# JiangongChen/ORB_SLAM3-1

Measured on AMD Instinct MI355X. Metric: tracking frames/s (ORB extract+match), higher is better.
Workload: dtype u8; 1 GPU; ORBextractor 640x480, 8 levels, 1000 features (configs[1]) + SearchByBoW 1000x1000 per frame (configs[2]); batch_per_gpu=256

## Files before the change

orb_slam3-1_amd/csrc/orbx_extractor.hip:

```cpp
#include <hip/hip_runtime.h>

#include <algorithm>
#include <cmath>
#include <cstdarg>
#include <cstdio>
#include <cstdlib>
#include <cstring>
#include <string>
#include <vector>

#include "hip_check.h"
#include "orbx_kernels.hip"

namespace orbx {

thread_local std::string g_last_error;

int fail(int code, const char* fmt, ...)
{
    char buf[512];
    va_list ap;
    va_start(ap, fmt);
    vsnprintf(buf, sizeof(buf), fmt, ap);
    va_end(ap);
// ... 37 lines not shown
        return ORBX_OK;
    }
    int upload(const std::vector<T>& v)
    {
        int r = ensure(v.size() ? v.size() : 1);
        if (r) return r;
        if (!v.empty()) ORBX_HIP(hipMemcpy(p, v.data(), v.size() * sizeof(T), hipMemcpyHostToDevice));
        return ORBX_OK;
    }
    void release() { if (p) (void)hipFree(p); p = nullptr; n = 0; }
};

}

using namespace orbx;

struct orbx_extractor {
    int device = 0;
    int nfeatures = 0, nlevels = 0, ini_th = 0, min_th = 0;
    float scale_factor_f = 0;
    double scale_factor_d = 0;
    std::vector<float> scale, inv_scale, sigma2, inv_sigma2;
    std::vector<int> nfeat;
    int taps[7];
    int max_kp = 0;

    int geo_w = 0, geo_h = 0;
    std::vector<LevelDesc> levels;
    std::vector<CellDesc> cells;
    std::vector<TileDesc> tiles;
    size_t pyr_frame_bytes = 0;
    int cand_frame_entries = 0, sel_frame_entries = 0;
    std::vector<StripDesc> strips;
    FastLds fast_layout;
    int fast_corner_cap = 0;
    size_t fast_lds = 0, oct_lds = 0;
    int oct_pool = 0, oct_lds_keys = 0, oct_small_keys = 0;
    bool oct_nodes_hbm = false;
    size_t oct_node_stride = 0;
    size_t oct_small_lds = 0;
    int oct_dyn_keys = 0;
    size_t oct_dyn_lds = 0;
    bool oct_keys_forced = false;

    DevBuf<LevelDesc> d_levels;
    DevBuf<CellDesc> d_cells;
    DevBuf<TileDesc> d_tiles;
    DevBuf<StripDesc> d_strips;
    std::vector<DevBuf<int> > d_qsx0;
    std::vector<DevBuf<uint4> > d_qsel, d_qalpha;
    std::vector<DevBuf<ResizeRow> > d_rows;
    std::vector<DevBuf<int> > d_xofs, d_yofs;
    std::vector<DevBuf<short> > d_ialpha, d_ibeta;
    std::vector<uint8_t> resize_generic;

    int batch_cap = 0, last_batch = 0;
    DevBuf<uint8_t> d_pyr, d_blur;
    DevBuf<uint32_t> d_cand, d_scratch, d_sel;
    DevBuf<uint8_t> d_oct_nodes;
    DevBuf<int> d_cell_count, d_sel_count, d_kp_dst;
    DevBuf<OrbxKeyPoint> d_lvl_kps;
    DevBuf<OrbxKeyPoint> d_kps;
    DevBuf<uint8_t> d_desc;
    DevBuf<int> d_n, d_mono, d_status;
    DevBuf<int> d_sad;
    DevBuf<uint8_t> d_stereo_io;
    int out_cap = 0;
    hipStream_t stream = nullptr;
    static constexpr int kProfEvents = 8;
    bool profile = false;
    hipEvent_t prof_ev[kProfEvents] = {};
    int prof_marks = 0;
    hipStream_t prof_stream = nullptr;
    hipStream_t side_stream = nullptr;
    hipEvent_t ev_fork = nullptr, ev_join = nullptr;
    hipStream_t oct_stream = nullptr;
    hipEvent_t ev_oct_join = nullptr, ev_fast0 = nullptr, ev_resize = nullptr;
    hipEvent_t ev_tail = nullptr;
    int dbg_tail_delay_us = 0;
    int last_octree_variant = 0;
    int oct_split = 0, oct_pool_hi = 0;
// ... 20 lines not shown
{
    const int nl = e->nlevels;
    e->scale.assign(nl, 1.0f); e->sigma2.assign(nl, 1.0f); e->inv_scale.resize(nl); e->inv_sigma2.resize(nl);
    for (int i = 1; i < nl; i++) {
        e->scale[i] = (float)(e->scale[i - 1] * e->scale_factor_d);
        e->sigma2[i] = e->scale[i] * e->scale[i];
    }
    for (int i = 0; i < nl; i++) {
        e->inv_scale[i] = 1.0f / e->scale[i];
        e->inv_sigma2[i] = 1.0f / e->sigma2[i];
    }
    e->nfeat.resize(nl);
    const float factor = (float)(1.0f / e->scale_factor_d);
    float per_scale = e->nfeatures * (1 - factor) / (1 - (float)std::pow((double)factor, (double)nl));
    int sum = 0;
    for (int l = 0; l < nl - 1; l++) {
        e->nfeat[l] = (int)std::nearbyintf(per_scale);
        sum += e->nfeat[l];
        per_scale *= factor;
    }
    e->nfeat[nl - 1] = std::max(e->nfeatures - sum, 0);
    e->max_kp = 0;
    for (int l = 0; l < nl; l++) e->max_kp += std::max(e->nfeat[l] + 3, 32);
    gauss_taps_q8(7, 2.0, e->taps);
}

int orbx_extractor::setup_geometry(int w, int h)
{
    if (w == geo_w && h == geo_h) return ORBX_OK;
    levels.assign(nlevels, LevelDesc());
    cells.clear();
    tiles.clear();
    strips.clear();
    size_t off = 0;
    int cand_off = 0, sel_off = 0, max_tw = 0, max_th = 0, max_nfeat = 0;
    std::vector<int> node_need(nlevels, 0);
    d_qsx0.resize(nlevels); d_yofs.resize(nlevels); d_qsel.resize(nlevels); d_qalpha.resize(nlevels); d_ibeta.resize(nlevels); d_rows.resize(nlevels);
    d_xofs.resize(nlevels); d_ialpha.resize(nlevels); resize_generic.assign(nlevels, 0);
    for (int l = 0; l < nlevels; l++) {
        LevelDesc& L = levels[l];
        L.w = (int)std::nearbyintf((float)w * inv_scale[l]);
        L.h = (int)std::nearbyintf((float)h * inv_scale[l]);
        if (L.w < 1 || L.h < 1) return fail(ORBX_ERR_ARG, "pyramid level %d of a %dx%d image is empty", l, w, h);
        if (L.w > 4096 + 32 || L.h > 4096 + 32) return fail(ORBX_ERR_ARG, "image %dx%d too large (keys are 12-bit)", w, h);
        L.stride = round_up(L.w, 64);
        L.off = (int64_t)off;
        off += (size_t)L.stride * L.h;
        off = (off + 255) & ~(size_t)255;
        L.nfeat = nfeat[l];
        L.scale = scale[l];
        L.patch_size = (int)(kPatch * scale[l]);
        {
            const int bw = (L.w - kEdge + 3) - (kEdge - 3), bh = (L.h - kEdge + 3) - (kEdge - 3);
            const int n_ini = bh > 0 ? (int)std::roundf((float)bw / (float)bh) : 0;
            L.sel_off = sel_off; L.sel_cap = std::max({nfeat[l] + 3, 32, 4 * std::max(n_ini, 0)});
            node_need[l] = std::max(nfeat[l], 4 * std::max(n_ini, 0));
        }
        sel_off += (L.sel_cap + 1) & ~1;
        max_nfeat = std::max(max_nfeat, node_need[l]);
        L.cell_begin = (int)cells.size();
        L.cand_off = cand_off;
        const int minBX = kEdge - 3, minBY = minBX, maxBX = L.w - kEdge + 3, maxBY = L.h - kEdge + 3;
        const float width = (float)(maxBX - minBX), height = (float)(maxBY - minBY);
        const int nCols = (int)(width / 35.f), nRows = (int)(height / 35.f);
        if (nCols > 0 && nRows > 0) {
            const int wCell = (int)std::ceil(width / nCols), hCell = (int)std::ceil(height / nRows);
// ... 99 lines not shown
                rows[dy].sy = (uint32_t)sy0 | ((uint32_t)sy1 << 16);
                rows[dy].b0 = (uint32_t)ib[2 * y] << 12; rows[dy].b1 = (uint32_t)ib[2 * y + 1] << 12; rows[dy].pad = 0;
            }
            int r;
            if (resize_generic[l] && ((r = d_xofs[l].upload(xofs)) || (r = d_ialpha[l].upload(ia)) || (r = d_yofs[l].upload(yofs)) || (r = d_ibeta[l].upload(ib)))) return r;
            if ((r = d_qsx0[l].upload(qsx0)) || (r = d_qsel[l].upload(qsel)) || (r = d_qalpha[l].upload(qal)) || (r = d_rows[l].upload(rows))) return r;
        }
    }
    pyr_frame_bytes = off;
    if (off >= ((size_t)1 << 31)) return fail(ORBX_ERR_ARG, "the pyramid of a %dx%d image exceeds 2 GiB per frame", w, h);
    cand_frame_entries = std::max(cand_off, 1);
    sel_frame_entries = sel_off;
    {
        if (cells.size() > 32767) return fail(ORBX_ERR_ARG, "%zu FAST cells exceed the strip table's 16-bit cell index", cells.size());
        int max_nch = 1, max_ngx = 1, max_sth = 7, max_ent = 1, max_ncell = 1, max_int = 1;
        for (const StripDesc& sd : strips) {
            const int g0 = (sd.x0 + 3) >> 2, g1 = (sd.x1 - 4) >> 2, ngx = g1 - g0 + 1, sth = sd.y1 - sd.y0, ih = sth - 6;
            if (ngx > 64 || ih > 127) return fail(ORBX_ERR_ARG, "FAST strip of %dx%d px exceeds the 64-quad x 127-row work item index", sd.x1 - sd.x0, sth);
            const int xa = (4 * (g0 - 1)) & ~15, qoff = 4 * g0 - xa;
            max_nch = std::max(max_nch, (qoff + 4 * ngx + 4 + 15) >> 4);
            for (int j = 0; j < sd.ncell; j++) { const CellDesc& c = cells[sd.cell0 + j]; max_int = std::max(max_int, (c.x1 - c.x0 - 6) * ih); }
            max_ngx = std::max(max_ngx, ngx); max_sth = std::max(max_sth, sth);
            max_ent = std::max(max_ent, ((ih + 3) / 4) * (ngx + sd.ncell - 1));
            max_ncell = std::max(max_ncell, (int)sd.ncell);
        }
        if (max_int > 8191) return fail(ORBX_ERR_ARG, "FAST cell interior of %d px exceeds the 8191-px bitmask", max_int);
        FastLds& Z = fast_layout;
        auto al16 = [](size_t v) { return (v + 15) & ~(size_t)15; };
        size_t o = 0;
        Z.tile_pitch = 16 * max_nch;
        o = al16((size_t)max_sth * Z.tile_pitch);
        Z.map_off = (int)o; Z.map_pitch = 4 * max_ngx + 8;
        o = al16(o + (size_t)(max_sth - 6 + 2) * Z.map_pitch);
        Z.colcell_off = (int)o; o = al16(o + Z.map_pitch);
        Z.ent_cap = (max_ent + 7) & ~7;
        Z.ent_off = (int)o; o = al16(o + 2 * 4 * (size_t)Z.ent_cap);
        Z.px_off = (int)o; o = al16(o + 2 * 4 * (size_t)kPxCap);
        Z.corner_cap = fast_corner_cap > 0 ? fast_corner_cap : kCornerCap;
        Z.corner_off = (int)o; o = al16(o + 2 * 4 * (size_t)Z.corner_cap);
        Z.wpc = (max_int + 31) / 32;
        Z.pre_off = (int)o; o = al16(o + 4 * (size_t)max_ncell * Z.wpc);
        Z.bits_off = (int)o; o = al16(o + 4 * (size_t)max_ncell * Z.wpc);
        Z.total = (int)o;
        fast_lds = o;
        if (fast_lds > 150 * 1024) return fail(ORBX_ERR_ARG, "FAST strip of %d quads x %d rows does not fit LDS", max_ngx, max_sth);
    }
    oct_pool = max_nfeat + 16;
    if (oct_pool > 32000) return fail(ORBX_ERR_ARG, "nfeatures per level %d too large for the device octree (16-bit node ids)", max_nfeat);
    const char* env = getenv("ORBX_OCT_LDS_KEYS");
    oct_lds_keys = env ? atoi(env) : 0;
    oct_keys_forced = env != nullptr;
    auto pool_bytes = [](int pool) { return (size_t)pool * (2 * sizeof(SortNode) + 8 + 16 + 2 * kOctLogFactor) + (size_t)((pool + 15) & ~15); };
    const size_t node_bytes = pool_bytes(oct_pool);
    oct_split = 0; oct_pool_hi = 0; oct_lds_hi = 0;
    {
        size_t best = (size_t)nlevels * node_bytes;
        for (int sp = 1; sp < nlevels; sp++) {
            int hi = 0;
            for (int l = sp; l < nlevels; l++) hi = std::max(hi, node_need[l]);
            const size_t cost = (size_t)sp * node_bytes + (size_t)(nlevels - sp) * pool_bytes(hi + 16);
            if (cost < best) { best = cost; oct_split = sp; oct_pool_hi = hi + 16; oct_lds_hi = pool_bytes(hi + 16) + 16; }
        }
    }
    oct_nodes_hbm = node_bytes > 150 * 1024;
    oct_node_stride = (node_bytes + 255) & ~(size_t)255;
    if (oct_nodes_hbm) oct_lds_keys = 0;
    if (!oct_nodes_hbm && node_bytes + 8 * (size_t)oct_lds_keys > 150 * 1024) oct_lds_keys = (int)((150 * 1024 - node_bytes) / 8);
    if (oct_lds_keys < 0) oct_lds_keys = 0;
    oct_lds = node_bytes + 8 * (size_t)oct_lds_keys + 16;
    int max_cand_cap = 0;
    for (const LevelDesc& lv : levels) max_cand_cap = std::max(max_cand_cap, lv.cand_cap);
    oct_small_keys = max_cand_cap;
    if (oct_nodes_hbm || node_bytes + 8 * (size_t)oct_small_keys > 150 * 1024) oct_small_keys = 0;
    oct_small_lds = node_bytes + 8 * (size_t)oct_small_keys + 16;
    if (oct_lds_keys > 0 && oct_lds_keys < max_cand_cap) oct_lds_keys = 0;
    oct_dyn_keys = 0; oct_dyn_lds = 0;
    if (!oct_nodes_hbm && oct_small_keys == 0 && node_bytes + 8 * 2048 <= 150 * 1024) {
        oct_dyn_keys = (int)std::min<size_t>((size_t)max_cand_cap, (150 * 1024 - node_bytes) / 8);
        if (const char* envd = getenv("ORBX_OCT_DYN_KEYS")) oct_dyn_keys = std::max(64, std::min(oct_dyn_keys, atoi(envd)));
        oct_dyn_lds = node_bytes + 8 * (size_t)oct_dyn_keys + 16;
    }
    if (!oct_nodes_hbm) {
        ORBX_HIP(hipFuncSetAttribute((const void*)k_octree<false>, hipFuncAttributeMaxDynamicSharedMemorySize, (int)node_bytes + 64));
        ORBX_HIP(hipFuncSetAttribute((const void*)k_octree<true>, hipFuncAttributeMaxDynamicSharedMemorySize, (int)std::max(oct_lds, oct_small_lds)));
        if (oct_dyn_keys > 0) ORBX_HIP(hipFuncSetAttribute((const void*)k_octree_dyn, hipFuncAttributeMaxDynamicSharedMemorySize, (int)oct_dyn_lds));
    } else {
        oct_lds = 64; oct_small_lds = 64;
    }
    ORBX_HIP(hipFuncSetAttribute((const void*)k_fast_strips, hipFuncAttributeMaxDynamicSharedMemorySize, (int)fast_lds));
    int r;
    if ((r = d_levels.upload(levels)) || (r = d_cells.upload(cells)) || (r = d_tiles.upload(tiles)) || (r = d_strips.upload(strips))) return r;
    geo_w = w; geo_h = h;
    batch_cap = 0;
    return ORBX_OK;
}

int orbx_extractor::ensure_batch(int batch)
{
    if (batch <= batch_cap) return ORBX_OK;
    int r;
    const size_t B = (size_t)batch;
    if ((r = d_pyr.ensure(B * pyr_frame_bytes + 64)) || (r = d_blur.ensure(B * pyr_frame_bytes + 64)) ||
        (r = d_cand.ensure(B * cand_frame_entries)) || (r = d_scratch.ensure(B * 2 * cand_frame_entries)) ||
        (r = d_sel.ensure(B * sel_frame_entries)) || (r = d_cell_count.ensure(B * std::max<size_t>(cells.size(), 1))) ||
        (r = d_sel_count.ensure(B * nlevels)) || (r = d_kp_dst.ensure(B * sel_frame_entries)) ||
        (r = d_lvl_kps.ensure(B * sel_frame_entries)) || (r = d_n.ensure(B)) || (r = d_mono.ensure(B)) || (r = d_status.ensure(B)))
        return r;
    if (oct_nodes_hbm && (r = d_oct_nodes.ensure(B * nlevels * oct_node_stride))) return r;
    ORBX_HIP(hipMemset(d_pyr.p, 0, B * pyr_frame_bytes + 64));
    ORBX_HIP(hipMemset(d_blur.p, 0, B * pyr_frame_bytes + 64));
    batch_cap = batch;
    return ORBX_OK;
}

namespace orbx {
__global__ void k_debug_spin(long long ticks)
{
    const long long t0 = wall_clock64();
    while (wall_clock64() - t0 < ticks) __builtin_amdgcn_s_sleep(32);
}
__global__ __launch_bounds__(256) void k_copy_level0(const uint8_t* __restrict__ src, int row_stride, size_t src_frame_stride,
                                                     uint8_t* __restrict__ pyr, size_t frame_stride, LevelDesc L)
{
    const int x4 = (blockIdx.x * blockDim.x + threadIdx.x) * 4;
    const int y = blockIdx.y;
    if (x4 >= L.w) return;
    const uint8_t* s = src + (size_t)blockIdx.z * src_frame_stride + (size_t)y * row_stride + x4;
    uint32_t v = 0;
#pragma unroll
    for (int k = 0; k < 4; k++) if (x4 + k < L.w) v |= (uint32_t)s[k] << (8 * k);
    *(uint32_t*)(pyr + (size_t)blockIdx.z * frame_stride + L.off + (size_t)y * L.stride + x4) = v;
}
}

int orbx_extractor::enqueue(const uint8_t* d_imgs, bool level0_ready, int batch, int row_stride, size_t frame_stride,
                            int lap0, int lap1, OrbxKeyPoint* o_kps, uint8_t* o_desc, int cap, int* o_n, int* o_mono, int* o_status,
                            hipStream_t st)
{
    const int B = batch;
    ORBX_HIP(hipMemsetAsync(o_status, 0, sizeof(int) * B, st));
    int mark_i = 0;
    auto mark = [&]() { if (profile && mark_i < kProfEvents) (void)hipEventRecord(prof_ev[mark_i++], st); };
#define ORBX_LAUNCHED(name) do { const hipError_t le_ = hipGetLastError(); if (le_ != hipSuccess) return fail(ORBX_ERR_HIP, "launch of %s: %s", name, hipGetErrorString(le_)); } while (0)
    const bool in_place = !level0_ready && ((uintptr_t)d_imgs % 16 == 0) && (row_stride % 16 == 0) && (frame_stride % 16 == 0);
    const int n_cells = (int)cells.size();
    const int quads = (sel_frame_entries + 7) / 8;

    auto run_range = [&](int f0, int nB, hipStream_t s, hipStream_t blur_s, bool marks) -> int {
        uint8_t* pyr = d_pyr.p + (size_t)f0 * pyr_frame_bytes;
        uint8_t* blr = d_blur.p + (size_t)f0 * pyr_frame_bytes;
        SrcImage lvl0;
        lvl0.base = nullptr; lvl0.frame_stride = 0; lvl0.stride = 0; lvl0.w = levels[0].w; lvl0.h = levels[0].h;
        if (in_place) { lvl0.base = d_imgs + (size_t)f0 * frame_stride; lvl0.frame_stride = frame_stride; lvl0.stride = row_stride; }
        if (marks) mark();
        if (!level0_ready && !in_place) {
            const LevelDesc& L0 = levels[0];
            dim3 g((L0.w / 4 + 255) / 256, L0.h, nB);
            hipLaunchKernelGGL(k_copy_level0, g, dim3(256), 0, s, d_imgs + (size_t)f0 * frame_stride, row_stride, frame_stride, pyr, pyr_frame_bytes, L0);
            ORBX_LAUNCHED("k_copy_level0");
        }
        if (marks) mark();
        int l_tail = (nB >= 64 && resize_tail_first >= 2 && resize_tail_first < nlevels) ? resize_tail_first : nlevels;
        for (int l = l_tail; l < nlevels; l++) if (resize_generic[l]) l_tail = nlevels;
        const bool chain_beside = resize_beside && blur_s && oct_stream && n_cells > 0 && l_tail < nlevels && l_tail > 1 &&
                                  !strips.empty() && strips[0].level == 0;
        hipStream_t rs = chain_beside ? oct_stream : s;
        if (chain_beside) { ORBX_HIP(hipEventRecord(ev_fork, s)); ORBX_HIP(hipStreamWaitEvent(rs, ev_fork, 0)); }
        for (int l = 1; l < l_tail; l++) {
            const LevelDesc& D = levels[l];
            dim3 g(xcd_grid(((D.w + kResizeTW - 1) / kResizeTW) * ((D.h + kResizeRows - 1) / kResizeRows)), nB);
            const LevelDesc& P = levels[l - 1];
            SrcImage src;
            src.base = pyr + P.off; src.frame_stride = pyr_frame_bytes; src.stride = P.stride; src.w = P.w; src.h = P.h;
            if (l == 1 && in_place) src = lvl0;
            if (resize_generic[l])
                hipLaunchKernelGGL(k_resize_generic, dim3((D.w + 255) / 256, D.h, nB), dim3(256), 0, rs, src, pyr, pyr_frame_bytes, D,
                                   d_xofs[l].p, d_ialpha[l].p, d_yofs[l].p, d_ibeta[l].p);
// ... 1 lines not shown
            hipLaunchKernelGGL(k_resize, g, dim3(256), 0, rs, src, pyr, pyr_frame_bytes, D,
                               d_qsx0[l].p, d_qsel[l].p, d_qalpha[l].p, d_rows[l].p);
            ORBX_LAUNCHED("k_resize");
        }
        if (chain_beside) ORBX_HIP(hipEventRecord(ev_resize, rs));
        const bool small_batch = !oct_keys_forced && oct_small_keys > 0 && (long long)B * nlevels <= 512;
        const bool dyn_keys = !oct_keys_forced && !small_batch && oct_dyn_keys > 0 && B <= oct_dyn_max_batch && !oct_dyn_off;
        const int dyn_k = (blur_s && B >= 32) ? std::min(oct_dyn_keys, oct_dyn_keys_beside) : oct_dyn_keys;
        const size_t o_lds = small_batch ? oct_small_lds : (dyn_keys ? oct_dyn_lds - 8 * (size_t)(oct_dyn_keys - dyn_k) : oct_lds);
        const int o_keys = small_batch ? oct_small_keys : (dyn_keys ? dyn_k : oct_lds_keys);
        uint32_t* sel = d_sel.p + (size_t)f0 * sel_frame_entries;
        int* sel_cnt = d_sel_count.p + (size_t)f0 * nlevels;
        int* kp_dst = d_kp_dst.p + (size_t)f0 * sel_frame_entries;
        auto oct_kernel = oct_nodes_hbm ? k_octree<false, false> : (dyn_keys ? k_octree_dyn : (o_keys > 0 ? k_octree<true, true> : k_octree<false, true>));
        const bool two_launches = !oct_nodes_hbm && (o_keys == 0 || dyn_keys) && oct_split > 0 && oct_stream && blur_s;
        const int lv_lo = two_launches ? oct_split : nlevels;
        auto launch_octree = [&](hipStream_t qs, int lv0, int lv1, size_t lds, int pool, int keys) {
            if (lv1 > lv0)
                hipLaunchKernelGGL(oct_kernel, dim3(lv1 - lv0, nB), dim3(64), lds, qs, d_levels.p, d_cells.p, d_cand.p + (size_t)f0 * cand_frame_entries, (size_t)cand_frame_entries,
                                   d_cell_count.p + (size_t)f0 * std::max<size_t>(cells.size(), 1), n_cells, d_scratch.p + (size_t)f0 * 2 * cand_frame_entries, (size_t)2 * cand_frame_entries, pool, keys,
                                   sel, sel_frame_entries, sel_cnt, nlevels, o_status + f0,
                                   d_oct_nodes.p ? d_oct_nodes.p + (size_t)f0 * nlevels * oct_node_stride : nullptr, oct_node_stride, lv0);
        };
        auto launch_blur = [&](hipStream_t bs) {
            hipLaunchKernelGGL(k_blur, dim3(xcd_grid((int)tiles.size()), nB), dim3(256), 0, bs, lvl0, pyr, in_place ? pyr : nullptr, blr, pyr_frame_bytes,
                               d_levels.p, d_tiles.p, (int)tiles.size(), taps[0], taps[1], taps[2], taps[3]);
        };
        bool oct0_early = false;
        bool tail_beside = false;
        uint32_t* cand = d_cand.p + (size_t)f0 * cand_frame_entries;
        int* cell_cnt = d_cell_count.p + (size_t)f0 * std::max<size_t>(cells.size(), 1);
        auto launch_fast = [&](hipStream_t fs, int s0, int s1) {
            if (s1 > s0)
                hipLaunchKernelGGL(k_fast_strips, dim3(xcd_grid(s1 - s0), nB), dim3(256), fast_lds, fs, lvl0, pyr, pyr_frame_bytes, d_levels.p, d_cells.p,
                                   d_strips.p + s0, s1 - s0, n_cells, ini_th, min_th, fast_layout, cand, (size_t)cand_frame_entries, cell_cnt);
        };
        int tail_strip = (int)strips.size();
        for (int si = (int)strips.size() - 1; si >= 0 && strips[si].level >= l_tail; si--) tail_strip = si;
        if (l_tail < nlevels) {
            ResizeTables T;
            std::memset(&T, 0, sizeof(T));
            for (int l = l_tail; l < nlevels; l++) { T.q_sx0[l] = d_qsx0[l].p; T.q_sel[l] = d_qsel[l].p; T.q_alpha[l] = d_qalpha[l].p; T.rows[l] = d_rows[l].p; }
            const bool beside = blur_s && oct_stream && n_cells > 0 && tail_strip > 0;
            hipStream_t ts = beside ? oct_stream : s;
            if (beside && !chain_beside) { ORBX_HIP(hipEventRecord(ev_fork, s)); ORBX_HIP(hipStreamWaitEvent(ts, ev_fork, 0)); }
            if (dbg_tail_delay_us > 0) hipLaunchKernelGGL(k_debug_spin, dim3(1), dim3(64), 0, ts, (long long)dbg_tail_delay_us * 100);
            hipLaunchKernelGGL(k_resize_tail, dim3(nB), dim3(1024), 0, ts, pyr, pyr_frame_bytes, d_levels.p, T, l_tail, nlevels);
            ORBX_LAUNCHED("k_resize_tail");
            if (beside) {
                ORBX_HIP(hipEventRecord(ev_tail, ts));
                tail_beside = true;
                launch_fast(ts, tail_strip, (int)strips.size());
                ORBX_HIP(hipEventRecord(ev_oct_join, ts));
                int l1_strip = tail_strip;
                for (int si = tail_strip - 1; si >= 0 && strips[si].level >= 1; si--) l1_strip = si;
                if (two_launches && oct_split > 1 && l1_strip > 0 && l1_strip < tail_strip) {
                    launch_fast(s, 0, l1_strip);
                    ORBX_HIP(hipEventRecord(ev_fast0, s));
                    ORBX_HIP(hipStreamWaitEvent(blur_s, ev_fast0, 0));
                    launch_octree(blur_s, 0, 1, o_lds, oct_pool, o_keys);
                    oct0_early = true;
                    if (chain_beside) ORBX_HIP(hipStreamWaitEvent(s, ev_resize, 0));
                    launch_fast(s, l1_strip, tail_strip);
                } else if (chain_beside && l1_strip > 0 && l1_strip < tail_strip) {
                    launch_fast(s, 0, l1_strip);
                    ORBX_HIP(hipStreamWaitEvent(s, ev_resize, 0));
                    launch_fast(s, l1_strip, tail_strip);
// ... 515 lines not shown
```

orb_slam3-1_amd/csrc/orbx_fast_strips.inc:

```

struct StripDesc {
    int16_t level;
    int16_t cell0, ncell;
    int16_t x0, x1;
    int16_t y0, y1;
    int16_t pad;
};

struct FastLds {
    int32_t tile_pitch;
    int32_t map_off, map_pitch;
    int32_t colcell_off;
    int32_t ent_off, ent_cap;
    int32_t px_off;
    int32_t corner_off, corner_cap;
    int32_t bits_off, pre_off, wpc;
    int32_t total;
};

constexpr int kStripMaxCells = 8;
constexpr int kStripWidth = 160;
constexpr int kEntBatch = 128;
constexpr int kPxCap = 4 * kEntBatch;
constexpr int kCornerCap = 256;

__device__ __forceinline__ int fast_m_tree(const uint8_t* __restrict__ t, int pitch)
{
    const int v = t[0];
    int d[16];
    d[0] = v - t[3 * pitch];       d[1] = v - t[3 * pitch + 1];   d[2] = v - t[2 * pitch + 2];   d[3] = v - t[pitch + 3];
    d[4] = v - t[3];               d[5] = v - t[-pitch + 3];      d[6] = v - t[-2 * pitch + 2];  d[7] = v - t[-3 * pitch + 1];
    d[8] = v - t[-3 * pitch];      d[9] = v - t[-3 * pitch - 1];  d[10] = v - t[-2 * pitch - 2]; d[11] = v - t[-pitch - 3];
    d[12] = v - t[-3];             d[13] = v - t[pitch - 3];      d[14] = v - t[2 * pitch - 2];  d[15] = v - t[3 * pitch - 1];
    int lo3[16], hi3[16];
#pragma unroll
    for (int k = 0; k < 16; k++) {
        lo3[k] = min(min(d[k], d[(k + 1) & 15]), d[(k + 2) & 15]);
        hi3[k] = max(max(d[k], d[(k + 1) & 15]), d[(k + 2) & 15]);
    }
    int best_dark = -256, best_bright = 256;
#pragma unroll
    for (int k = 0; k < 16; k++) {
        const int lo9 = min(min(lo3[k], lo3[(k + 3) & 15]), lo3[(k + 6) & 15]);
        const int hi9 = max(max(hi3[k], hi3[(k + 3) & 15]), hi3[(k + 6) & 15]);
        best_dark = max(best_dark, lo9);
        best_bright = min(best_bright, hi9);
    }
    return max(max(best_dark, -best_bright), 0);
}

__device__ __forceinline__ int wave_incl_scan(int v)
{
    v += __builtin_amdgcn_update_dpp(0, v, 0x111, 0xF, 0xF, false);
    v += __builtin_amdgcn_update_dpp(0, v, 0x112, 0xF, 0xF, false);
    v += __builtin_amdgcn_update_dpp(0, v, 0x114, 0xF, 0xF, false);
    v += __builtin_amdgcn_update_dpp(0, v, 0x118, 0xF, 0xF, false);
    v += __builtin_amdgcn_update_dpp(0, v, 0x142, 0xA, 0xF, false);
    v += __builtin_amdgcn_update_dpp(0, v, 0x143, 0xC, 0xF, false);
    return v;
}

__device__ __forceinline__ void wave_lds_fence()
{
    __builtin_amdgcn_fence(__ATOMIC_RELEASE, "wavefront");
    __builtin_amdgcn_wave_barrier();
    __builtin_amdgcn_fence(__ATOMIC_ACQUIRE, "wavefront");
}

#ifdef ORBX_FAST_TIMING
__device__ unsigned long long d_fast_prof[16];
#define ORBX_FTICK(k) if (threadIdx.x == 0) { const long long t_now = clock64(); atomicAdd(&d_fast_prof[(k) + fallback_slot], (unsigned long long)(t_now - t_prev)); t_prev = t_now; }
#else
#define ORBX_FTICK(k)
#endif
__global__ __launch_bounds__(256) void k_fast_strips(SrcImage lvl0, const uint8_t* __restrict__ pyr, size_t frame_stride,
                                                     const LevelDesc* __restrict__ levels, const CellDesc* __restrict__ cells,
                                                     const StripDesc* __restrict__ strips, int n_strips, int n_cells,
                                                     int ini_th, int min_th, FastLds Z,
                                                     uint32_t* __restrict__ cand, size_t cand_frame_stride, int* __restrict__ cell_count)
{
    extern __shared__ __align__(16) uint8_t smem[];
    __shared__ int s_cx0[kStripMaxCells], s_iw[kStripMaxCells], s_total[kStripMaxCells], s_slot_off[kStripMaxCells], s_slot_cap[kStripMaxCells];
    __shared__ int s_seg[4][kStripMaxCells + 1];
#ifdef ORBX_FAST_TIMING
    long long t_prev = clock64();
    int fallback_slot = 0;
#endif

    const int strip_idx = xcd_remap(blockIdx.x, gridDim.x, blockIdx.y);
    if (strip_idx >= n_strips) return;
    const StripDesc S = strips[strip_idx];
    const LevelDesc L = levels[S.level];
    const int frame = blockIdx.y;
#if defined(ORBX_FAST_CUT)
    if ((int)threadIdx.x < S.ncell) cell_count[(size_t)frame * n_cells + S.cell0 + threadIdx.x] = 0;
#endif
    const bool ext = S.level == 0 && lvl0.base != nullptr;
    const uint8_t* img = ext ? lvl0.base + (size_t)frame * lvl0.frame_stride : pyr + (size_t)frame * frame_stride + L.off;
    const int istride = ext ? lvl0.stride : L.stride;
    const int tid = threadIdx.x, lane = tid & 63, wave = __builtin_amdgcn_readfirstlane(tid >> 6);

    const int th = S.y1 - S.y0, ih = th - 6;
    const int g0 = (S.x0 + 3) >> 2, g1 = (S.x1 - 4) >> 2;
    const int ngx = g1 - g0 + 1;
    const int xa = (4 * (g0 - 1)) & ~15;
    const int qoff = 4 * g0 - xa;
    const int nch = (qoff + 4 * ngx + 4 + 15) >> 4;
    const int TP = Z.tile_pitch, MP = Z.map_pitch;
    uint8_t* tile = smem;
    uint8_t* mmap = smem + Z.map_off;
    uint8_t* colcell = smem + Z.colcell_off;
    uint16_t* ent = (uint16_t*)(smem + Z.ent_off) + wave * Z.ent_cap;
    uint16_t* pxl = (uint16_t*)(smem + Z.px_off) + wave * kPxCap;
    uint16_t* corners = (uint16_t*)(smem + Z.corner_off) + wave * Z.corner_cap;
    uint32_t* bits = (uint32_t*)(smem + Z.bits_off);
    uint32_t* pre = (uint32_t*)(smem + Z.pre_off);
    const int WPC = Z.wpc;

    {
        const float inv = 1.0f / (float)nch;
        for (int i = tid; i < th * nch; i += 256) {
            const int r = (int)(((float)i + 0.5f) * inv), q = i - r * nch;
            *(uint4*)(tile + r * TP + 16 * q) = *(const uint4*)(img + (size_t)(S.y0 + r) * istride + xa + 16 * q);
        }
    }
    for (int i = tid; i < ((ih + 2) * MP) >> 2; i += 256) ((uint32_t*)mmap)[i] = 0u;
    for (int i = tid; i < S.ncell * WPC; i += 256) bits[i] = 0u;
    for (int i = tid; i < MP; i += 256) colcell[i] = 0xFF;
    if (tid < S.ncell) {
        const CellDesc c = cells[S.cell0 + tid];
        s_cx0[tid] = c.x0 + 3 - 4 * g0 + 4; s_iw[tid] = c.x1 - c.x0 - 6;
        s_slot_off[tid] = c.slot_off; s_slot_cap[tid] = c.slot_cap;
    }
    __syncthreads();
    for (int j = 0; j < S.ncell; j++)
        for (int i = tid; i < s_iw[j]; i += 256) colcell[s_cx0[j] + i] = (uint8_t)j;
    __syncthreads();

    ORBX_FTICK(0)
#if defined(ORBX_FAST_CUT) && ORBX_FAST_CUT == 0
    return;
#endif
    auto nms_pixel = [&](const int y, const int mc, const int t, const int cA, const int cB) {
        const uint8_t* p = mmap + (y + 1) * MP + mc;
        const int m = p[0];
        const int j = colcell[mc];
        if (m > t && j >= cA && j < cB) {
            const int xl = mc - s_cx0[j], iw = s_iw[j];
            const bool hl = xl > 0, hr = xl < iw - 1, hu = y > 0, hd = y < ih - 1;
            const int r0 = p[-MP - 1], r1 = p[-MP], r2 = p[-MP + 1], r3 = p[-1], r4 = p[1], r5 = p[MP - 1], r6 = p[MP], r7 = p[MP + 1];
            const int n0 = (hu && hl) ? r0 : 0, n1 = hu ? r1 : 0, n2 = (hu && hr) ? r2 : 0;
            const int n3 = hl ? r3 : 0, n4 = hr ? r4 : 0;
            const int n5 = (hd && hl) ? r5 : 0, n6 = hd ? r6 : 0, n7 = (hd && hr) ? r7 : 0;
            const int nmax = max(max(max(n0, n1), max(n2, n3)), max(max(n4, n5), max(n6, n7)));
            const bool keep = (m - 1) > ((nmax > t) ? nmax - 1 : 0);
            if (keep) { const int q = y * iw + xl; atomicOr(&bits[j * WPC + (q >> 5)], 1u << (q & 31)); }
        }
    };
    auto emit_pixel = [&](const int y, const int mc, const int cA, const int cB) {
        const int j = colcell[mc];
        if (j >= cA && j < cB) {
            const int iw = s_iw[j], q = y * iw + (mc - s_cx0[j]);
            const uint32_t wd = bits[j * WPC + (q >> 5)];
            if ((wd >> (q & 31)) & 1u) {
                const int rk = (int)pre[j * WPC + (q >> 5)] + __popc(wd & ((1u << (q & 31)) - 1u));
                const int m = mmap[(y + 1) * MP + mc];
                if (rk < s_slot_cap[j])
                    cand[(size_t)frame * cand_frame_stride + s_slot_off[j] + rk] =
                        pack_key((uint32_t)(4 * g0 + mc - 4 - 16), (uint32_t)(S.y0 + 3 + y - 16), (uint32_t)(m - 1));
            }
        }
    };

    int ncorner = 0;
    int gA = 0, ng = 1;

    auto set_cols = [&](const int cA, const int cB) {
        const int mA = s_cx0[cA], mB = s_cx0[cB - 1] + s_iw[cB - 1] - 1;
        gA = (mA - 4) >> 2;
        ng = ((mB - 4) >> 2) - gA + 1;
    };
    const int nrow_w = (ih - wave + 3) >> 2;
    auto stage1 = [&](const int t, int nent) {
        const int n_items = nrow_w * ng;
        {
            const uint32_t T2 = (uint32_t)t | ((uint32_t)t << 16);
            const int q64 = 64 / ng, r64 = 64 - q64 * ng;
            int ry = (int)(((float)lane + 0.5f) * (1.0f / (float)ng)), gx = lane - ry * ng;
            for (int base = 0; base < n_items; base += 64) {
                uint32_t entry = 0;
                if (base + lane < n_items) {
                    const int y = 4 * ry + wave;
                    const uint32_t* row = (const uint32_t*)(tile + (y + 3) * TP + qoff) + gA + gx;
                    const int pd = TP >> 2;
                    const uint32_t cur = row[0], prv = row[-1], nxt = row[1], up3 = row[-3 * pd], dn3 = row[3 * pd];
                    const us2 ce = as_us2(__builtin_amdgcn_perm(0u, cur, 0x0C020C00u)), co = as_us2(__builtin_amdgcn_perm(0u, cur, 0x0C030C01u));
                    const us2 r0e = as_us2(__builtin_amdgcn_perm(0u, dn3, 0x0C020C00u)), r0o = as_us2(__builtin_amdgcn_perm(0u, dn3, 0x0C030C01u));
                    const us2 r8e = as_us2(__builtin_amdgcn_perm(0u, up3, 0x0C020C00u)), r8o = as_us2(__builtin_amdgcn_perm(0u, up3, 0x0C030C01u));
                    const us2 r4e = as_us2(__builtin_amdgcn_perm(nxt, cur, 0x0C050C03u)), r4o = as_us2(__builtin_amdgcn_perm(nxt, cur, 0x0C060C04u));
                    const us2 r12e = as_us2(__builtin_amdgcn_perm(cur, prv, 0x0C030C01u)), r12o = as_us2(__builtin_amdgcn_perm(cur, prv, 0x0C040C02u));
                    const us2 T2v = as_us2(T2);
                    const us2 lo_e = __builtin_elementwise_sub_sat(ce, T2v), lo_o = __builtin_elementwise_sub_sat(co, T2v);
                    const us2 hi_e = ce + T2v, hi_o = co + T2v;
                    const us2 dk_e = __builtin_elementwise_max(__builtin_elementwise_min(r0e, r8e), __builtin_elementwise_min(r4e, r12e));
                    const us2 dk_o = __builtin_elementwise_max(__builtin_elementwise_min(r0o, r8o), __builtin_elementwise_min(r4o, r12o));
                    const us2 br_e = __builtin_elementwise_min(__builtin_elementwise_max(r0e, r8e), __builtin_elementwise_max(r4e, r12e));
                    const us2 br_o = __builtin_elementwise_min(__builtin_elementwise_max(r0o, r8o), __builtin_elementwise_max(r4o, r12o));
                    const uint32_t c_e = as_u32(__builtin_elementwise_sub_sat(lo_e, dk_e)) | as_u32(__builtin_elementwise_sub_sat(br_e, hi_e));
                    const uint32_t c_o = as_u32(__builtin_elementwise_sub_sat(lo_o, dk_o)) | as_u32(__builtin_elementwise_sub_sat(br_o, hi_o));
                    uint32_t m_e, m_o;
                    asm("v_pk_min_u16 %0, %1, %2" : "=v"(m_e) : "v"(c_e), "v"(0x00010001u));
// ... 40 lines not shown
                int id = 0;
                if (i < npx) {
                    id = pxl[i];
                    const int y = id >> 8, xq = (id & 0xFF) + 4 * gA;
                    id = (y << 8) | xq;
                    const int m = fast_m_tree(tile + (y + 3) * TP + qoff + xq, TP);
                    mmap[(y + 1) * MP + xq + 4] = (uint8_t)m;
                    corner = m > t;
                }
                const unsigned long long bal = __ballot(corner);
                const int at = ncorner + (int)__builtin_amdgcn_mbcnt_hi((uint32_t)(bal >> 32), __builtin_amdgcn_mbcnt_lo((uint32_t)bal, 0u));
                if (corner && at < Z.corner_cap) corners[at] = (uint16_t)id;
                ncorner += __popcll(bal);
            }
            wave_lds_fence();
        }
    };
    auto for_corners = [&](const int y0, const int ystep, const int nrows, auto&& fn) {
        if (ncorner <= Z.corner_cap) {
            for (int base = 0; base < ncorner; base += 64) {
                const int i = base + lane;
                if (i < ncorner) { const int id = corners[i]; fn(id >> 8, (id & 0xFF) + 4); }
            }
        } else {
            const int wpx = 4 * ng, n = nrows * wpx;
            const float inv = 1.0f / (float)wpx;
            for (int i = lane; i < n; i += 64) {
                const int ry = (int)(((float)i + 0.5f) * inv), xq = 4 * gA + i - ry * wpx;
                fn(ystep * ry + y0, xq + 4);
            }
        }
    };
    auto rank_cell = [&](const int j) {
        const int nwords = (s_iw[j] * ih + 31) >> 5;
        int run = 0;
        for (int w0 = 0; w0 < nwords; w0 += 64) {
            const int i = w0 + lane;
            const int my = (i < nwords) ? __popc(bits[j * WPC + i]) : 0;
            const int incl = wave_incl_scan(my);
            if (i < nwords) pre[j * WPC + i] = (uint32_t)(run + incl - my);
            run += __builtin_amdgcn_readlane(incl, 63);
        }
        if (lane == 0) s_total[j] = run;
    };
    uint32_t fb_cells = 0u;
    set_cols(0, S.ncell);
    {
        const int nent = stage1(ini_th, 0);
        ORBX_FTICK(1)
#if !defined(ORBX_FAST_CUT) || ORBX_FAST_CUT >= 2
        const int d = (wave * Z.ent_cap) | (wave << 16);
        stage2(ini_th, nent, nent, nent, nent, d, d, d, d);
#endif
    }
    ORBX_FTICK(2)
#if !defined(ORBX_FAST_CUT) || ORBX_FAST_CUT >= 3
    __syncthreads();
    ORBX_FTICK(3)
    for_corners(wave, 4, nrow_w, [&](int y, int mc) { nms_pixel(y, mc, ini_th, 0, S.ncell); });
    __syncthreads();
    ORBX_FTICK(4)
    for (int j = wave; j < S.ncell; j += 4) rank_cell(j);
    __syncthreads();
    ORBX_FTICK(5)
    fb_cells = (uint32_t)__ballot(lane < S.ncell && s_total[min(lane, kStripMaxCells - 1)] == 0);
    for_corners(wave, 4, nrow_w, [&](int y, int mc) { emit_pixel(y, mc, 0, S.ncell); });
    ORBX_FTICK(6)
#endif
#if defined(ORBX_FAST_CUT)
    if (ini_th >= 0) return;
#endif
#ifdef ORBX_FAST_TIMING
    fallback_slot = 8;
#endif
    if (fb_cells) {
        int k = 0, nent = 0;
        if (lane == 0) s_seg[wave][0] = 0;
        for (uint32_t rest = fb_cells; rest; rest &= rest - 1u, k++) {
            const int j = __builtin_ctz(rest);
            set_cols(j, j + 1);
            nent = stage1(min_th, nent);
            if (lane == 0) s_seg[wave][k + 1] = nent;
        }
        ORBX_FTICK(1)
        __syncthreads();
        ORBX_FTICK(3)
        k = 0;
        for (uint32_t rest = fb_cells; rest; rest &= rest - 1u, k++) {
            if ((k & 3) != wave) continue;
            const int j = __builtin_ctz(rest);
#ifdef ORBX_FAST_TIMING
            if (threadIdx.x == 0) atomicAdd(&d_fast_prof[15], 1ull);
#endif
            set_cols(j, j + 1);
            auto seg = [&](int w, int kk) { return __builtin_amdgcn_readfirstlane(s_seg[w][kk]); };
            const int b0 = seg(0, k), b1 = seg(1, k), b2 = seg(2, k), b3 = seg(3, k);
            const int c1 = seg(0, k + 1) - b0, c2 = c1 + seg(1, k + 1) - b1, c3 = c2 + seg(2, k + 1) - b2, n = c3 + seg(3, k + 1) - b3;
            const int d0 = b0, d1 = (Z.ent_cap + b1 - c1) | (1 << 16), d2 = (2 * Z.ent_cap + b2 - c2) | (2 << 16), d3 = (3 * Z.ent_cap + b3 - c3) | (3 << 16);
            ncorner = 0;
            stage2(min_th, n, c1, c2, c3, d0, d1, d2, d3);
            ORBX_FTICK(2)
            for_corners(0, 1, ih, [&](int y, int mc) { nms_pixel(y, mc, min_th, j, j + 1); });
            wave_lds_fence();
            ORBX_FTICK(4)
            rank_cell(j);
            wave_lds_fence();
            ORBX_FTICK(5)
            for_corners(0, 1, ih, [&](int y, int mc) { emit_pixel(y, mc, j, j + 1); });
            ORBX_FTICK(6)
        }
    }
    __syncthreads();
    if (tid < S.ncell) cell_count[(size_t)frame * n_cells + S.cell0 + tid] = min(s_total[tid], s_slot_cap[tid]);
}
```

Measured before the change: 271,200 frames/s.

## Precompute per-strip FAST records on host and batch tile loads in kernel prologue

Per-strip geometry, cell offsets and the column-to-cell map are now precomputed on the host into a single packed StripRec. The FAST strip kernel loads it with a few vector reads instead of dereferencing level and cell descriptors and building the colcell table in LDS behind an extra barrier. The tile load now uses exact reciprocal integer division and issues three 16-byte global loads per thread before any LDS store, to expose more memory-level parallelism. Zeroing also moves to 16-byte stores. In exchange, strip records grow by a fixed table, and in-place input gets a new stride limit.

```diff
diff --git a/orb_slam3-1_amd/csrc/orbx_extractor.hip b/orb_slam3-1_amd/csrc/orbx_extractor.hip
--- a/orb_slam3-1_amd/csrc/orbx_extractor.hip
+++ b/orb_slam3-1_amd/csrc/orbx_extractor.hip
@@ -93,6 +93,7 @@
     size_t pyr_frame_bytes = 0;
     int cand_frame_entries = 0, sel_frame_entries = 0;
     std::vector<StripDesc> strips;
+    std::vector<StripRec> strip_recs;
     FastLds fast_layout;
     int fast_corner_cap = 0;
     size_t fast_lds = 0, oct_lds = 0;
@@ -107,7 +108,7 @@
     DevBuf<LevelDesc> d_levels;
     DevBuf<CellDesc> d_cells;
     DevBuf<TileDesc> d_tiles;
-    DevBuf<StripDesc> d_strips;
+    DevBuf<StripRec> d_strips;
     std::vector<DevBuf<int> > d_qsx0;
     std::vector<DevBuf<uint4> > d_qsel, d_qalpha;
     std::vector<DevBuf<ResizeRow> > d_rows;
@@ -194,6 +195,7 @@
     cells.clear();
     tiles.clear();
     strips.clear();
+    strip_recs.clear();
     size_t off = 0;
     int cand_off = 0, sel_off = 0, max_tw = 0, max_th = 0, max_nfeat = 0;
     std::vector<int> node_need(nlevels, 0);
@@ -359,7 +361,6 @@
         o = al16((size_t)max_sth * Z.tile_pitch);
         Z.map_off = (int)o; Z.map_pitch = 4 * max_ngx + 8;
         o = al16(o + (size_t)(max_sth - 6 + 2) * Z.map_pitch);
-        Z.colcell_off = (int)o; o = al16(o + Z.map_pitch);
         Z.ent_cap = (max_ent + 7) & ~7;
         Z.ent_off = (int)o; o = al16(o + 2 * 4 * (size_t)Z.ent_cap);
         Z.px_off = (int)o; o = al16(o + 2 * 4 * (size_t)kPxCap);
@@ -371,6 +372,33 @@
         Z.total = (int)o;
         fast_lds = o;
         if (fast_lds > 150 * 1024) return fail(ORBX_ERR_ARG, "FAST strip of %d quads x %d rows does not fit LDS", max_ngx, max_sth);
+        strip_recs.assign(strips.size(), StripRec());
+        for (size_t si = 0; si < strips.size(); si++) {
+            const StripDesc& sd = strips[si];
+            const LevelDesc& L = levels[sd.level];
+            StripRec& R = strip_recs[si];
+            const int g0 = (sd.x0 + 3) >> 2, g1 = (sd.x1 - 4) >> 2, ngx = g1 - g0 + 1;
+            const int xa = (4 * (g0 - 1)) & ~15, qoff = 4 * g0 - xa, nch = (qoff + 4 * ngx + 4 + 15) >> 4, sth = sd.y1 - sd.y0;
+            R.src_off = (uint32_t)((size_t)L.off + (size_t)sd.y0 * L.stride + xa);
+            R.stride = (uint32_t)L.stride;
+            auto pair = [](int lo, int hi) { return (uint32_t)lo | ((uint32_t)hi << 16); };
+            if (sd.y0 < 0 || xa < 0 || sd.cell0 < 0) return fail(ORBX_ERR_INTERNAL, "FAST strip at row %d, column %d, cell %d", sd.y0, xa, sd.cell0);
+            R.y0_xa = pair(sd.y0, xa); R.th_nch = pair(sth, nch); R.g0_qoff = pair(g0, qoff); R.ncell_cell0 = pair(sd.ncell, sd.cell0);
+            R.level = (uint32_t)sd.level;
+            R.inv_nch = (65536u + (uint32_t)nch - 1u) / (uint32_t)nch;
+            for (uint32_t i = 0; i < (uint32_t)(sth * nch); i++)
+                if (((i * R.inv_nch) >> 16) != i / (uint32_t)nch)
+                    return fail(ORBX_ERR_INTERNAL, "FAST strip of %d rows x %d chunks: the row of chunk %u is not exact", sth, nch, i);
+            std::memset(R.tab.colcell, 0xFF, sizeof(R.tab.colcell));
+            for (int j = 0; j < sd.ncell; j++) {
+                const CellDesc& c = cells[sd.cell0 + j];
+                R.tab.cx0[j] = c.x0 + 3 - 4 * g0 + 4; R.tab.iw[j] = c.x1 - c.x0 - 6;
+                R.tab.slot_off[j] = c.slot_off; R.tab.slot_cap[j] = c.slot_cap;
+                if (R.tab.cx0[j] < 0 || R.tab.cx0[j] + R.tab.iw[j] > Z.map_pitch)
+                    return fail(ORBX_ERR_INTERNAL, "FAST cell columns %d + %d outside the strip's %d map columns", R.tab.cx0[j], R.tab.iw[j], Z.map_pitch);
+                for (int i = 0; i < R.tab.iw[j]; i++) R.tab.colcell[R.tab.cx0[j] + i] = (uint8_t)j;
+            }
+        }
     }
     oct_pool = max_nfeat + 16;
     if (oct_pool > 32000) return fail(ORBX_ERR_ARG, "nfeatures per level %d too large for the device octree (16-bit node ids)", max_nfeat);
@@ -416,7 +444,7 @@
     }
     ORBX_HIP(hipFuncSetAttribute((const void*)k_fast_strips, hipFuncAttributeMaxDynamicSharedMemorySize, (int)fast_lds));
     int r;
-    if ((r = d_levels.upload(levels)) || (r = d_cells.upload(cells)) || (r = d_tiles.upload(tiles)) || (r = d_strips.upload(strips))) return r;
+    if ((r = d_levels.upload(levels)) || (r = d_cells.upload(cells)) || (r = d_tiles.upload(tiles)) || (r = d_strips.upload(strip_recs))) return r;
     geo_w = w; geo_h = h;
     batch_cap = 0;
     return ORBX_OK;
@@ -469,7 +497,7 @@
     int mark_i = 0;
     auto mark = [&]() { if (profile && mark_i < kProfEvents) (void)hipEventRecord(prof_ev[mark_i++], st); };
 #define ORBX_LAUNCHED(name) do { const hipError_t le_ = hipGetLastError(); if (le_ != hipSuccess) return fail(ORBX_ERR_HIP, "launch of %s: %s", name, hipGetErrorString(le_)); } while (0)
-    const bool in_place = !level0_ready && ((uintptr_t)d_imgs % 16 == 0) && (row_stride % 16 == 0) && (frame_stride % 16 == 0);
+    const bool in_place = !level0_ready && ((uintptr_t)d_imgs % 16 == 0) && (row_stride % 16 == 0) && (frame_stride % 16 == 0) && row_stride < (1 << 23);
     const int n_cells = (int)cells.size();
     const int quads = (sel_frame_entries + 7) / 8;
 
@@ -537,7 +565,7 @@
         int* cell_cnt = d_cell_count.p + (size_t)f0 * std::max<size_t>(cells.size(), 1);
         auto launch_fast = [&](hipStream_t fs, int s0, int s1) {
             if (s1 > s0)
-                hipLaunchKernelGGL(k_fast_strips, dim3(xcd_grid(s1 - s0), nB), dim3(256), fast_lds, fs, lvl0, pyr, pyr_frame_bytes, d_levels.p, d_cells.p,
+                hipLaunchKernelGGL(k_fast_strips, dim3(xcd_grid(s1 - s0), nB), dim3(256), fast_lds, fs, lvl0, pyr, pyr_frame_bytes,
                                    d_strips.p + s0, s1 - s0, n_cells, ini_th, min_th, fast_layout, cand, (size_t)cand_frame_entries, cell_cnt);
         };
         int tail_strip = (int)strips.size();
diff --git a/orb_slam3-1_amd/csrc/orbx_fast_strips.inc b/orb_slam3-1_amd/csrc/orbx_fast_strips.inc
--- a/orb_slam3-1_amd/csrc/orbx_fast_strips.inc
+++ b/orb_slam3-1_amd/csrc/orbx_fast_strips.inc
@@ -7,10 +7,33 @@
     int16_t pad;
 };
 
+constexpr int kStripMaxCells = 8;
+constexpr int kStripMapPitchMax = 4 * 64 + 8;
+
+struct __attribute__((aligned(16))) StripTab {
+    int32_t cx0[kStripMaxCells];
+    int32_t iw[kStripMaxCells];
+    int32_t slot_off[kStripMaxCells], slot_cap[kStripMaxCells];
+    uint8_t colcell[(kStripMapPitchMax + 15) & ~15];
+};
+
+struct __attribute__((aligned(16))) StripRec {
+    uint32_t src_off;
+    uint32_t stride;
+    uint32_t y0_xa;
+    uint32_t th_nch;
+    uint32_t g0_qoff;
+    uint32_t ncell_cell0;
+    uint32_t level;
+    uint32_t inv_nch;
+    StripTab tab;
+};
+static_assert(sizeof(StripTab) % 16 == 0 && sizeof(StripRec) == 32 + sizeof(StripTab), "StripRec: 32 header bytes, then the table");
+constexpr int kStripTabChunks = (int)(sizeof(StripTab) / 16);
+
 struct FastLds {
     int32_t tile_pitch;
     int32_t map_off, map_pitch;
-    int32_t colcell_off;
     int32_t ent_off, ent_cap;
     int32_t px_off;
     int32_t corner_off, corner_cap;
@@ -18,7 +41,6 @@
     int32_t total;
 };
 
-constexpr int kStripMaxCells = 8;
 constexpr int kStripWidth = 160;
 constexpr int kEntBatch = 128;
 constexpr int kPxCap = 4 * kEntBatch;
@@ -74,13 +96,13 @@
 #define ORBX_FTICK(k)
 #endif
 __global__ __launch_bounds__(256) void k_fast_strips(SrcImage lvl0, const uint8_t* __restrict__ pyr, size_t frame_stride,
-                                                     const LevelDesc* __restrict__ levels, const CellDesc* __restrict__ cells,
-                                                     const StripDesc* __restrict__ strips, int n_strips, int n_cells,
+                                                     const StripRec* __restrict__ recs, int n_strips, int n_cells,
                                                      int ini_th, int min_th, FastLds Z,
                                                      uint32_t* __restrict__ cand, size_t cand_frame_stride, int* __restrict__ cell_count)
 {
     extern __shared__ __align__(16) uint8_t smem[];
-    __shared__ int s_cx0[kStripMaxCells], s_iw[kStripMaxCells], s_total[kStripMaxCells], s_slot_off[kStripMaxCells], s_slot_cap[kStripMaxCells];
+    __shared__ StripTab s_tab;
+    __shared__ int s_total[kStripMaxCells];
     __shared__ int s_seg[4][kStripMaxCells + 1];
 #ifdef ORBX_FAST_TIMING
     long long t_prev = clock64();
@@ -89,27 +111,28 @@
 
     const int strip_idx = xcd_remap(blockIdx.x, gridDim.x, blockIdx.y);
     if (strip_idx >= n_strips) return;
-    const StripDesc S = strips[strip_idx];
-    const LevelDesc L = levels[S.level];
+    const StripRec* S = recs + strip_idx;
     const int frame = blockIdx.y;
+    const int tid = threadIdx.x, lane = tid & 63, wave = __builtin_amdgcn_readfirstlane(tid >> 6);
+    const uint4 h0 = ((const uint4*)S)[0], h1 = ((const uint4*)S)[1];
+    uint4 tab_chunk = make_uint4(0u, 0u, 0u, 0u);
+    if (wave == 0) tab_chunk = ((const uint4*)&S->tab)[min(lane, kStripTabChunks - 1)];
+    const int sy0 = (int)(h0.z & 0xFFFFu), xa = (int)(h0.z >> 16);
+    const int th = (int)(h0.w & 0xFFFFu), nch = (int)(h0.w >> 16), ih = th - 6;
+    const int g0 = (int)(h1.x & 0xFFFFu), qoff = (int)(h1.x >> 16);
+    const int ncell = (int)(h1.y & 0xFFFFu), cell0 = (int)(h1.y >> 16);
+    const uint32_t inv_nch = h1.w;
 #if defined(ORBX_FAST_CUT)
-    if ((int)threadIdx.x < S.ncell) cell_count[(size_t)frame * n_cells + S.cell0 + threadIdx.x] = 0;
-#endif
-    const bool ext = S.level == 0 && lvl0.base != nullptr;
-    const uint8_t* img = ext ? lvl0.base + (size_t)frame * lvl0.frame_stride : pyr + (size_t)frame * frame_stride + L.off;
-    const int istride = ext ? lvl0.stride : L.stride;
-    const int tid = threadIdx.x, lane = tid & 63, wave = __builtin_amdgcn_readfirstlane(tid >> 6);
-
-    const int th = S.y1 - S.y0, ih = th - 6;
-    const int g0 = (S.x0 + 3) >> 2, g1 = (S.x1 - 4) >> 2;
-    const int ngx = g1 - g0 + 1;
-    const int xa = (4 * (g0 - 1)) & ~15;
-    const int qoff = 4 * g0 - xa;
-    const int nch = (qoff + 4 * ngx + 4 + 15) >> 4;
+    if ((int)threadIdx.x < ncell) cell_count[(size_t)frame * n_cells + cell0 + threadIdx.x] = 0;
+#endif
+    const bool ext = h1.z == 0u && lvl0.base != nullptr;
+    const uint8_t* img = (ext ? lvl0.base : pyr) + (size_t)frame * (ext ? lvl0.frame_stride : frame_stride) +
+                         (ext ? (size_t)sy0 * (size_t)lvl0.stride + (size_t)xa : (size_t)h0.x);
+    const uint32_t istride = ext ? (uint32_t)lvl0.stride : h0.y;
+
     const int TP = Z.tile_pitch, MP = Z.map_pitch;
     uint8_t* tile = smem;
     uint8_t* mmap = smem + Z.map_off;
-    uint8_t* colcell = smem + Z.colcell_off;
     uint16_t* ent = (uint16_t*)(smem + Z.ent_off) + wave * Z.ent_cap;
     uint16_t* pxl = (uint16_t*)(smem + Z.px_off) + wave * kPxCap;
     uint16_t* corners = (uint16_t*)(smem + Z.corner_off) + wave * Z.corner_cap;
@@ -117,24 +140,28 @@
     uint32_t* pre = (uint32_t*)(smem + Z.pre_off);
     const int WPC = Z.wpc;
 
+    const int n_chunk = th * nch;
+    uint4 c0, c1, c2;
+    uint32_t d0, d1, d2;
+    auto issue = [&](const int k, uint32_t& dst) {
+        const uint32_t i = (uint32_t)min(tid + 256 * k, n_chunk - 1);
+        const uint32_t r = __umul24(i, inv_nch) >> 16, q = i - __umul24(r, (uint32_t)nch);
+        dst = __umul24(r, (uint32_t)TP) + 16u * q;
+        return *(const uint4*)(img + (__umul24(r, istride) + 16u * q));
+    };
+    auto land = [&](const int k, const uint32_t dst, const uint4& c) { if (tid + 256 * k < n_chunk) *(uint4*)(tile + dst) = c; };
+    c0 = issue(0, d0); c1 = issue(1, d1); c2 = issue(2, d2);
     {
-        const float inv = 1.0f / (float)nch;
-        for (int i = tid; i < th * nch; i += 256) {
-            const int r = (int)(((float)i + 0.5f) * inv), q = i - r * nch;
-            *(uint4*)(tile + r * TP + 16 * q) = *(const uint4*)(img + (size_t)(S.y0 + r) * istride + xa + 16 * q);
-        }
-    }
-    for (int i = tid; i < ((ih + 2) * MP) >> 2; i += 256) ((uint32_t*)mmap)[i] = 0u;
-    for (int i = tid; i < S.ncell * WPC; i += 256) bits[i] = 0u;
-    for (int i = tid; i < MP; i += 256) colcell[i] = 0xFF;
-    if (tid < S.ncell) {
-        const CellDesc c = cells[S.cell0 + tid];
-        s_cx0[tid] = c.x0 + 3 - 4 * g0 + 4; s_iw[tid] = c.x1 - c.x0 - 6;
-        s_slot_off[tid] = c.slot_off; s_slot_cap[tid] = c.slot_cap;
-    }
-    __syncthreads();
-    for (int j = 0; j < S.ncell; j++)
-        for (int i = tid; i < s_iw[j]; i += 256) colcell[s_cx0[j] + i] = (uint8_t)j;
+        const uint4 zero = make_uint4(0u, 0u, 0u, 0u);
+        for (int i = tid; i < ((ih + 2) * MP + 15) >> 4; i += 256) ((uint4*)mmap)[i] = zero;
+        for (int i = tid; i < (ncell * WPC + 3) >> 2; i += 256) ((uint4*)bits)[i] = zero;
+    }
+    if (wave == 0 && lane < kStripTabChunks) ((uint4*)&s_tab)[lane] = tab_chunk;
+    land(0, d0, c0); land(1, d1, c1); land(2, d2, c2);
+    for (int k = 3; 256 * k < n_chunk; k += 3) {
+        c0 = issue(k, d0); c1 = issue(k + 1, d1); c2 = issue(k + 2, d2);
+        land(k, d0, c0); land(k + 1, d1, c1); land(k + 2, d2, c2);
+    }
     __syncthreads();
 
     ORBX_FTICK(0)
@@ -144,9 +171,9 @@
     auto nms_pixel = [&](const int y, const int mc, const int t, const int cA, const int cB) {
         const uint8_t* p = mmap + (y + 1) * MP + mc;
         const int m = p[0];
-        const int j = colcell[mc];
+        const int j = s_tab.colcell[mc];
         if (m > t && j >= cA && j < cB) {
-            const int xl = mc - s_cx0[j], iw = s_iw[j];
+            const int xl = mc - s_tab.cx0[j], iw = s_tab.iw[j];
             const bool hl = xl > 0, hr = xl < iw - 1, hu = y > 0, hd = y < ih - 1;
             const int r0 = p[-MP - 1], r1 = p[-MP], r2 = p[-MP + 1], r3 = p[-1], r4 = p[1], r5 = p[MP - 1], r6 = p[MP], r7 = p[MP + 1];
             const int n0 = (hu && hl) ? r0 : 0, n1 = hu ? r1 : 0, n2 = (hu && hr) ? r2 : 0;
@@ -158,16 +185,16 @@
         }
     };
     auto emit_pixel = [&](const int y, const int mc, const int cA, const int cB) {
-        const int j = colcell[mc];
+        const int j = s_tab.colcell[mc];
         if (j >= cA && j < cB) {
-            const int iw = s_iw[j], q = y * iw + (mc - s_cx0[j]);
+            const int iw = s_tab.iw[j], q = y * iw + (mc - s_tab.cx0[j]);
             const uint32_t wd = bits[j * WPC + (q >> 5)];
             if ((wd >> (q & 31)) & 1u) {
                 const int rk = (int)pre[j * WPC + (q >> 5)] + __popc(wd & ((1u << (q & 31)) - 1u));
                 const int m = mmap[(y + 1) * MP + mc];
-                if (rk < s_slot_cap[j])
-                    cand[(size_t)frame * cand_frame_stride + s_slot_off[j] + rk] =
-                        pack_key((uint32_t)(4 * g0 + mc - 4 - 16), (uint32_t)(S.y0 + 3 + y - 16), (uint32_t)(m - 1));
+                if (rk < s_tab.slot_cap[j])
+                    cand[(size_t)frame * cand_frame_stride + s_tab.slot_off[j] + rk] =
+                        pack_key((uint32_t)(4 * g0 + mc - 4 - 16), (uint32_t)(sy0 + 3 + y - 16), (uint32_t)(m - 1));
             }
         }
     };
@@ -176,7 +203,7 @@
     int gA = 0, ng = 1;
 
     auto set_cols = [&](const int cA, const int cB) {
-        const int mA = s_cx0[cA], mB = s_cx0[cB - 1] + s_iw[cB - 1] - 1;
+        const int mA = s_tab.cx0[cA], mB = s_tab.cx0[cB - 1] + s_tab.iw[cB - 1] - 1;
         gA = (mA - 4) >> 2;
         ng = ((mB - 4) >> 2) - gA + 1;
     };
@@ -283,7 +310,7 @@
         }
     };
     auto rank_cell = [&](const int j) {
-        const int nwords = (s_iw[j] * ih + 31) >> 5;
+        const int nwords = (s_tab.iw[j] * ih + 31) >> 5;
         int run = 0;
         for (int w0 = 0; w0 < nwords; w0 += 64) {
             const int i = w0 + lane;
@@ -295,7 +322,7 @@
         if (lane == 0) s_total[j] = run;
     };
     uint32_t fb_cells = 0u;
-    set_cols(0, S.ncell);
+    set_cols(0, ncell);
     {
         const int nent = stage1(ini_th, 0);
         ORBX_FTICK(1)
@@ -308,14 +335,14 @@
 #if !defined(ORBX_FAST_CUT) || ORBX_FAST_CUT >= 3
     __syncthreads();
     ORBX_FTICK(3)
-    for_corners(wave, 4, nrow_w, [&](int y, int mc) { nms_pixel(y, mc, ini_th, 0, S.ncell); });
+    for_corners(wave, 4, nrow_w, [&](int y, int mc) { nms_pixel(y, mc, ini_th, 0, ncell); });
     __syncthreads();
     ORBX_FTICK(4)
-    for (int j = wave; j < S.ncell; j += 4) rank_cell(j);
+    for (int j = wave; j < ncell; j += 4) rank_cell(j);
     __syncthreads();
     ORBX_FTICK(5)
-    fb_cells = (uint32_t)__ballot(lane < S.ncell && s_total[min(lane, kStripMaxCells - 1)] == 0);
-    for_corners(wave, 4, nrow_w, [&](int y, int mc) { emit_pixel(y, mc, 0, S.ncell); });
+    fb_cells = (uint32_t)__ballot(lane < ncell && s_total[min(lane, kStripMaxCells - 1)] == 0);
+    for_corners(wave, 4, nrow_w, [&](int y, int mc) { emit_pixel(y, mc, 0, ncell); });
     ORBX_FTICK(6)
 #endif
 #if defined(ORBX_FAST_CUT)
@@ -362,5 +389,5 @@
         }
     }
     __syncthreads();
-    if (tid < S.ncell) cell_count[(size_t)frame * n_cells + S.cell0 + tid] = min(s_total[tid], s_slot_cap[tid]);
+    if (tid < ncell) cell_count[(size_t)frame * n_cells + cell0 + tid] = min(s_total[tid], s_tab.slot_cap[tid]);
 }
```

New measurement: 281,800 frames/s (median of 6 runs). 3.9% higher.
